# tomas-gr/RawNanoporeSignalCompression

Hardware: AMD Instinct MI355X
Metric: MSamples/s encode+decode (1/2/4/8 GPU) at fixed ratio; % HBM roofline (higher is better)
Workload: dtype int16; 1 GPU; configs[1]: 100000 reads x 100000 int16 samples per GPU (1 chunk each), C5 encode+decode; reads_per_gpu=100000, samples_per_read=100000, global_reads=100000, parallelism=dp1 (reads round-robin, no data-path collective)

## Files before the change

rawnanoporesignalcompression_amd/csrc/pgn_kernels.hip:

```cpp
#include <hip/hip_runtime.h>
#include <stdio.h>
#include <stdlib.h>
#include <string.h>

#include <algorithm>
#include <condition_variable>
#include <mutex>
#include <vector>

#include "../../include/pgnano_hip.h"
#include "../../include/pgnano_pod5.h"
#include "pgn_c5.h"
#include "pgn_internal.h"
#include "pgn_segment.h"
#include "pgn_stitch.h"
#include "pgn_ctc.h"
#include "pgn_crf.h"
#include "pgn_crf_post.h"
#include "pgn_qual.h"
#include "pgn_select.h"
#include "pgn_vbz.h"
#include "pgn_variants.h"
#include "pgn_zdec.h"
#include "pgn_zenc.h"
// ... 477 lines not shown
    bool ex = tot <= kAllocLimit;
    for (int s = 0; ex && s < nf; s++) {
        const int64_t b = z1::frame_content_bound(src + fo[s], (size_t)fl[s]);
        ex = b >= 0 && (uint64_t)b >= cs[s];
    }
    *sum = tot;
    *maxClaim = mx;
    *expand = ex;
    return true;
}
__host__ __device__ inline bool claims_pass_chunk(const uint8_t* src, uint64_t len, int nf, uint32_t n, uint64_t* sum)
{
    uint64_t mx = 0;
    bool ex = false;
    if (!blob_claims(src, len, nf, sum, &mx, &ex) || !ex) return false;
    return *sum + kVbzPadding > inter_cap(n) || mx > n;
}

__global__ void claim_scan_kernel(const uint8_t* in, const uint64_t* inOffsets, const uint64_t* inSizes,
                                  const uint32_t* counts, size_t n, int nf, uint32_t* list, uint32_t* hdr)
{
    for (size_t i = (size_t)blockIdx.x * blockDim.x + threadIdx.x; i < n; i += (size_t)gridDim.x * blockDim.x) {
        uint64_t sum = 0;
        if (!claims_pass_chunk(in + inOffsets[i], inSizes[i], nf, counts[i], &sum)) continue;
        list[atomicAdd(hdr + 4, 1u)] = (uint32_t)i;
        const uint64_t kib = (sum + 1023) >> 10;
        atomicMax(hdr + 5, kib < 0xFFFFFFFFull ? (uint32_t)kib : 0xFFFFFFFFu);
    }
}

__device__ inline int c5_parse_chunk(const uint8_t* in, uint64_t src0, uint64_t len, DecUnit* u, size_t interCap)
{
    const uint8_t* src = in + src0;
    uint64_t pos = 0;
    uint64_t cs[5];
    for (int s = 0; s < kStreams; s++) {
        uint64_t fl;
        if (s < 4) {
            if (pos > len || len - pos < 8) return PGN_ERR_CORRUPT;
            fl = ld64u(src + pos);
            pos += 8;
            if (fl > len - pos) return PGN_ERR_CORRUPT;
        } else {
            fl = len - pos;
        }
        bool ok = false;
        cs[s] = z1::frame_content_size(src + pos, (size_t)fl, &ok);
        if (!ok) return PGN_ERR_NOT_ZSTD;
        u[s].src = src0 + pos;
        u[s].len = (uint32_t)fl;
        pos += fl;
    }
    uint64_t off = 0;
    for (int s = 0; s < kStreams; s++) {
        if (cs[s] > kPassSamples || cs[s] > interCap - off) return over_claim_status(in, u, cs, kStreams);
        u[s].cs = (uint32_t)cs[s];
        u[s].interOff = (uint32_t)off;
        off += cs[s];
    }
    return PGN_OK;
}

__global__ __launch_bounds__(64) void dec_parse_kernel(DecArgs a)
{
    const size_t g = (size_t)blockIdx.x * 64 + lane_id();
    const size_t c = a.base + g;
    if (g >= a.G || c >= a.nchunks) return;
    a.status[c] = a.sampleCounts[c] > kPassSamples ? PGN_ERR_UNSUPPORTED
                                                   : c5_parse_chunk(a.in, a.inOffsets[c], a.inSizes[c], a.units + g * kStreams,
                                                                    inter_cap(a.capN));
}

__global__ __launch_bounds__(64) __attribute__((amdgpu_waves_per_eu(5))) void dec_zstd_kernel(DecArgs a)
{
    const int lane = lane_id();
    const DecLayout lay = dec_layout();
    uint8_t* sbase = a.slotScratch + (size_t)blockIdx.x * a.slotBytes;
    DecScratch S;
    S.lit = sbase + lay.lit;
    S.tables = (uint32_t*)(sbase + lay.tables);
    S.htab = (uint16_t*)(sbase + lay.htab);
    S.coopCmd = nullptr;
    S.coopStg = nullptr;
    PhaseProf P;
    P.init(a.prof);
    const size_t G = a.G, units = (size_t)a.nu * G;
    uint32_t tk = 0;
    if (lane == 0) tk = atomicAdd(a.queue, 1u);
    while (true) {
        const uint32_t u = __builtin_amdgcn_readfirstlane(tk);
        if (u >= units) break;
        if (lane == 0) tk = atomicAdd(a.queue, 1u);
        const int s = a.nu == 1 ? 0 : unit_stream((uint32_t)(u / G));
        const size_t g = u % G;
        const size_t c = a.base + g;
        S.job = a.jobs ? a.jobs + (g * kStreams + (size_t)s) * kJobBytes : nullptr;
        if (S.job && lane == 0) gst<uint32_t>(&((HufJob*)S.job)->flag, 0u);
        if (c >= a.nchunks || a.status[c] != PGN_OK) continue;
        DecUnit& d = a.units[g * kStreams + s];
        const size_t cap = a.nu == 1 ? (size_t)d.cs + kVbzPadding : (size_t)d.cs;
        uint8_t* const dst = a.inter + g * a.interStride + d.interOff;
        P.mark(3);
        long r = dec_frame_fast(a.in + d.src, d.len, dst, cap, S.job, S.htab, P, sDec.hb);
        P.mark(2);
        if (r < 0) r = zstd_decompress_wave(a.in + d.src, d.len, dst, cap, S, P);
        if (lane == 0) d.dres = (int32_t)r;
        wave_sync();
    }
    P.flush();
}

constexpr int kHufFrames = 16;
#ifndef PGN_K2_PF
#define PGN_K2_PF 1
#endif
constexpr uint32_t kPf = PGN_K2_PF;
constexpr uint32_t kRing = 16 * kPf;
constexpr uint32_t kRingBlocks = kRing / 4;
constexpr uint32_t kTabStride = kJobTabUse;
constexpr uint32_t kZeroTab = 16;
constexpr size_t kHufJunkBytes = 64 * 128;
static_assert((2 * kTabStride) % 16 == 0, "frame tables stay 16-byte aligned");

__device__ __forceinline__ uint64_t shl64(uint64_t c, uint32_t e)
{
    return c << (e & 63u);
}
__device__ __forceinline__ uint32_t cnd(bool c, uint32_t a, uint32_t b)
{
    uint32_t r;
    asm volatile("v_cndmask_b32 %0, %2, %1, %3" : "=v"(r) : "v"(a), "v"(b), "s"((uint64_t)ballot(c)));
    return r;
}
__device__ __forceinline__ uint32_t pick4(bool q1, bool q2, uint32_t a, uint32_t b, uint32_t c, uint32_t d)
{
    return cnd(q2, cnd(q1, d, c), cnd(q1, b, a));
}
__device__ __forceinline__ uint32_t sel4(const uint4& v, uint32_t i)
{
    return i == 0 ? v.x : (i == 1 ? v.y : (i == 2 ? v.z : v.w));
}

__global__ __launch_bounds__(64) void dec_huf_kernel(DecArgs a)
{
    __shared__ __attribute__((aligned(16))) uint16_t tabs[kHufFrames * kTabStride + kZeroTab];
    __shared__ uint32_t ring[kRing * 64];
    const uint32_t lane = (uint32_t)lane_id();
    const size_t G = a.G;
    const uint32_t ngrp = (uint32_t)((G + kHufFrames - 1) / kHufFrames);
    const uint32_t kq = blockIdx.x / ngrp;
    if (kq >= a.nu) return;
    const int s = unit_stream(kq);
    const size_t g0 = (size_t)(blockIdx.x % ngrp) * kHufFrames;
    const uint32_t f = lane >> 2, q = lane & 3;
    const size_t g = g0 + f;
    const bool inb = g < G && a.base + g < a.nchunks;
    const HufJob* J = (const HufJob*)(a.jobs + (inb ? (g * kStreams + (size_t)s) * kJobBytes : 0));
    const uint32_t flag = inb ? gld<uint32_t>(&J->flag) : 0u;
    const uint64_t fm = ballot(flag != 0);
    if (fm == 0) return;
    if (a.hufPrio) __builtin_amdgcn_s_setprio(3);
    PhaseProf Pp;
    Pp.init(a.prof ? a.prof + (kHufProfOff - kPhases) : nullptr);
    Pp.count(0);
    Pp.count(2, (uint64_t)__builtin_popcountll(fm));
    {
        const uint32_t lt = lane < kTabStride / 8 ? lane : kTabStride / 8 - 1;
        uint4 tv[kHufFrames];
#pragma unroll
        for (int ff = 0; ff < kHufFrames; ff++) {
            const size_t gf = (fm >> (4 * ff)) & 1u ? g0 + (size_t)ff : g0;
            tv[ff] = gld<uint4>(a.jobs + (gf * kStreams + (size_t)s) * kJobBytes + sizeof(HufJob) + 16 * lt);
        }
#pragma unroll
        for (int ff = 0; ff < kHufFrames; ff++)
            if (lane < kTabStride / 8) *(uint4*)&tabs[ff * kTabStride + 8 * lane] = tv[ff];
        if (lane < kZeroTab / 2) ((uint32_t*)&tabs[kHufFrames * kTabStride])[lane] = 0u;
    }
    uint8_t* const junk = a.jobs + G * kStreams * kJobBytes + 128 * lane;
    Pp.mark(0);
    uint64_t hp = 0, dstp = 0;
    uint4 len = make_uint4(0, 0, 0, 0), prm = make_uint4(0, 11, 0, 0);
    uint32_t C2 = 0;
    if (flag) {
        hp = gld<uint64_t>(&J->hp);
        dstp = gld<uint64_t>(&J->dst);
        len = gld<uint4>(&J->len[0]);
        prm = gld<uint4>(&J->rs);
        C2 = gld<uint32_t>(&J->C2);
    }
    const uint32_t rs = prm.x, tl = prm.y, d1 = prm.z & 0xFFu, d2 = prm.z >> 8, C1 = prm.w;
    const uint32_t so = (q > 0 ? len.x : 0u) + (q > 1 ? len.y : 0u) + (q > 2 ? len.z : 0u);
    const uint32_t sl = sel4(len, q);
    const uint32_t seg = (rs + 3) / 4;
    uint32_t nsym = flag ? (q == 3 ? rs - 3 * seg : seg) : 0u;
    const uint8_t* src = (const uint8_t*)hp + 6 + so;
    uint8_t* sdst = (uint8_t*)dstp + (size_t)seg * q;
    const uint32_t lastB = (flag && sl) ? (uint32_t)gb(src + sl - 1) : 0u;
    bool bad = flag && lastB == 0;
    const bool live = flag && !bad;
    if (!live) nsym = 0;
    const uint32_t sh1 = 32 - tl, shA = sh1 + d1, shB = sh1 + d2;
    const uint64_t e = live ? (uint64_t)src + sl - 1 : (uint64_t)junk;
    const uint64_t amin = live ? ((uint64_t)src & ~(uint64_t)15) : (uint64_t)junk;
    const uint64_t gtop = e & ~(uint64_t)15;
    const uint32_t bmax = (uint32_t)((gtop - amin) >> 4);
#if PGN_K2_DIAG == 2
    auto blk = [&](uint32_t b) { return gld<uint4>((const void*)(gtop - 16ull * (b < bmax ? b : bmax) * 0)); };
#else
    auto blk = [&](uint32_t b) { return gld<uint4>((const void*)(gtop - 16ull * (b < bmax ? b : bmax))); };
#endif
    auto stage = [&](uint32_t b, const uint4& v) {
        uint32_t* r = ring + lane + 256u * (b & (kRingBlocks - 1u));
        r[0] = v.w;
        r[64] = v.z;
        r[128] = v.y;
        r[192] = v.x;
    };
    const uint32_t hb = lastB ? z1::highbit32(lastB) : 0u;
    const uint32_t i0 = (uint32_t)(e >> 2) & 3u;
    const uint32_t v0 = live ? (uint32_t)(e & 3u) * 8u + hb : 0u;
    const uint32_t totalBits = sl ? (sl - 1) * 8u + hb : 0u;
    const uint32_t ins0 = 4 - i0;
    uint32_t insb = ins0 << 8, avail = v0;
    const uint32_t laneOff = 4u * lane;
    auto ring_at = [&](uint32_t ib) -> uint32_t {
        return *(const uint32_t*)((const uint8_t*)ring + ((ib & ((kRing - 1) << 8)) | laneOff));
    };
    uint64_t C;
    uint32_t nd;
    uint4 La[kPf], Lb[kPf];
    uint32_t lb[kPf];
    auto issue = [&](uint32_t slot) {
        lb[slot] = (insb >> 10) + 2 * kPf;
        La[slot] = blk(lb[slot]);
        Lb[slot] = blk(lb[slot] + 1);
    };
    {
        uint4 b0v[2 * kPf + 2];
#pragma unroll
        for (uint32_t k = 0; k < 2 * kPf + 2; k++) b0v[k] = blk(k);
#pragma unroll
        for (uint32_t k = 0; k < kPf; k++) {
            issue(k);
            gst<uint4>(junk, make_uint4(0, 0, 0, 0));
        }
#pragma unroll
        for (uint32_t k = 0; k < 2 * kPf + 2; k++) stage(k, b0v[k]);
        const uint4 b0 = b0v[0];
        const uint32_t dw0 = sel4(b0, i0);
        C = v0 ? ((uint64_t)dw0 << (64 - v0)) : 0ull;
        nd = ring_at(insb);
        C |= shl64((uint64_t)nd, 32u - avail);
        avail += 32;
        insb += 256;
        nd = ring_at(insb);
        if (avail <= 32) {
            C |= (uint64_t)nd;
            avail += 32;
            insb += 256;
            nd = ring_at(insb);
        }
    }
    uint64_t Cadd = 0;
    auto refill = [&]() {
        const uint32_t m01 = avail <= 32 ? 1u : 0u;
        const uint32_t x = m01 ? nd : 0u;
        Cadd = shl64((uint64_t)x, 32u - avail);
        avail += m01 << 5;
        insb += m01 << 8;
        nd = ring_at(insb);
    };
    const uint32_t tbLive = f * kTabStride, tbZero = kHufFrames * kTabStride;
    uint32_t tb = tbLive, tc1 = C1 + tbLive, tc2 = C2 + tbLive, s1 = sh1;
    auto symbol = [&](bool merge) -> uint32_t {
        const uint32_t hi = (uint32_t)(C >> 32);
        const uint32_t a0 = ((hi >> s1) + tb) << 1, a1 = ((hi >> shA) + tc1) << 1, a2 = ((hi >> shB) + tc2) << 1;
        const uint32_t am = a0 < a1 ? a0 : a1;
#if PGN_K2_DIAG == 3
        const uint32_t ent = ((am < a2 ? am : a2) & 0xFF00u) | (4u + (hi >> 30));
#else
        const uint32_t ent = *(const uint16_t*)((const uint8_t*)tabs + (am < a2 ? am : a2));
#endif
        C = shl64(merge ? (C | Cadd) : C, ent);
        avail -= ent & 0xFFu;
        return ent;
    };
    auto word4 = [&]() -> uint32_t {
        const uint32_t e0 = symbol(true);
        const uint32_t e1 = symbol(false);
        refill();
        const uint32_t e2 = symbol(true);
        const uint32_t e3 = symbol(false);
        refill();
        return __builtin_amdgcn_perm(e1, e0, 0x0C0C0501u) | __builtin_amdgcn_perm(e3, e2, 0x05010C0Cu);
    };
    auto freeze = [&](bool fz) {
        tb = fz ? tbZero : tbLive;
        tc1 = fz ? tbZero : C1 + tbLive;
        tc2 = fz ? tbZero : C2 + tbLive;
        s1 = fz ? 28u : sh1;
    };
    const uint32_t h = (16u - ((uint32_t)(uintptr_t)sdst & 15u)) & 15u;
    uint8_t* A0 = sdst + h;
    const uint32_t rb = h & 3u;
    const bool q1 = (h >> 2) & 1u, q2 = (h >> 3) & 1u;
    const uint32_t m0 = ((128u - ((uint32_t)(uintptr_t)A0 & 127u)) & 127u) >> 4;
    const int sft = 7 - (int)m0;
    const int sg = (int)(nsym / 16);
    const int nD = sg - 1;
    uint32_t P[4] = {0, 0, 0, 0}, F[4] = {0, 0, 0, 0};
    auto active = [&](int gi) { const int li = gi - sft; return li >= 0 && li < sg; };
    auto iteration = [&](int gi) -> uint4 {
        stage(lb[0], La[0]);
        stage(lb[0] + 1, Lb[0]);
#pragma unroll
        for (uint32_t k = 0; k + 1 < kPf; k++) {
            lb[k] = lb[k + 1];
            La[k] = La[k + 1];
            Lb[k] = Lb[k + 1];
        }
        issue(kPf - 1);
        uint32_t W[4];
#pragma unroll
        for (int k = 0; k < 4; k++) W[k] = word4();
        const uint32_t X0 = pick4(q1, q2, P[0], P[1], P[2], P[3]), X1 = pick4(q1, q2, P[1], P[2], P[3], W[0]),
                       X2 = pick4(q1, q2, P[2], P[3], W[0], W[1]), X3 = pick4(q1, q2, P[3], W[0], W[1], W[2]),
                       X4 = pick4(q1, q2, W[0], W[1], W[2], W[3]);
        const uint4 D = make_uint4(__builtin_amdgcn_alignbyte(X1, X0, rb), __builtin_amdgcn_alignbyte(X2, X1, rb),
                                   __builtin_amdgcn_alignbyte(X3, X2, rb), __builtin_amdgcn_alignbyte(X4, X3, rb));
        const bool act = active(gi);
        if (gi < 8) {
            const bool first = gi == sft;
#pragma unroll
            for (int k = 0; k < 4; k++) F[k] = cnd(first, W[k], F[k]);
        }
#pragma unroll
        for (int k = 0; k < 4; k++) P[k] = cnd(act, W[k], P[k]);
        freeze(!active(gi + 1));
        return D;
    };
    freeze(!active(0));
#pragma unroll
    for (int gi = 0; gi < 8; gi++) {
        const uint4 D = iteration(gi);
        const int m = gi - sft - 1;
#if PGN_K2_DIAG == 1
        uint8_t* ad = junk;
#else
        uint8_t* ad = (m >= 0 && m < nD) ? A0 + 16 * m : junk;
#endif
        gst<uint4>(ad, D);
    }
#pragma unroll
    for (int k = 1; k < 8; k++) gst<uint4>(junk + 16 * k, make_uint4(0, 0, 0, 0));
    const int lines = nD > (int)m0 ? (nD - (int)m0 + 7) / 8 : 0;
    const int trips = (int)wave_max((uint32_t)lines);
    Pp.mark(1);
    Pp.count(1, (uint64_t)trips);
    Pp.count(3, (uint64_t)wave_sum(nsym));
    for (int t = 0; t < trips; t++) {
        uint4 Dk[8];
#pragma unroll
        for (int k = 0; k < 8; k++) Dk[k] = iteration(8 + 8 * t + k);
#pragma unroll
        for (int k = 0; k < 8; k++) {
            const int m = (int)m0 + 8 * t + k;
#if PGN_K2_DIAG == 1
            uint8_t* ad = junk + 16 * k;
#else
            uint8_t* ad = m < nD ? A0 + 16 * m : junk + 16 * k;
#endif
            gst<uint4>(ad, Dk[k]);
        }
    }
    Pp.mark(2);
#pragma unroll
    for (uint32_t k = 0; k < kPf; k++) {
        stage(lb[k], La[k]);
        stage(lb[k] + 1, Lb[k]);
    }
    freeze(false);
    C |= Cadd;
    Cadd = 0;
    if (sg > 0) {
        for (uint32_t b = 0; b < h; b++) gst<uint8_t>(sdst + b, (uint8_t)(sel4(make_uint4(F[0], F[1], F[2], F[3]), b >> 2) >> (8 * (b & 3))));
        const uint32_t J16 = 16 * (uint32_t)sg - 16;
        for (uint32_t b = h; b < 16; b++)
            gst<uint8_t>(sdst + J16 + b, (uint8_t)(sel4(make_uint4(P[0], P[1], P[2], P[3]), b >> 2) >> (8 * (b & 3))));
    }
    for (uint32_t i = 16 * (uint32_t)sg; i < nsym; i++) {
        const uint32_t ent = symbol(true);
        refill();
        gst<uint8_t>(sdst + i, (uint8_t)(ent >> 8));
    }
    if (live) bad = (v0 + 32u * ((insb >> 8) - ins0) - avail) != totalBits;
    const uint64_t bm = ballot(bad);
    if (q == 0 && flag && ((bm >> (4 * f)) & 0xFull)) gst<int32_t>(&a.units[g * kStreams + (size_t)s].dres, (int32_t)z1::kDecErrHufStream);
    Pp.mark(3);
    Pp.flush();
}

__global__ __launch_bounds__(64 * kCoopWaves) void dec_huf_wide_kernel(DecArgs a)
{
    const uint32_t u = blockIdx.x;
    const size_t G = a.G;
    if ((size_t)u >= (size_t)a.nu * G) return;
    const int s = unit_stream((uint32_t)(u / G));
    const size_t g = u % G;
    if (a.base + g >= a.nchunks) return;
    const HufJob* J = (const HufJob*)(a.jobs + (g * kStreams + (size_t)s) * kJobBytes);
    if (gld<uint32_t>(&J->flag) == 0) return;
    __shared__ uint32_t stgAll[kCoopWaves * kCoopStgWords];
    __shared__ uint32_t bad;
    const uint32_t tid = threadIdx.x;
    const int wid = (int)__builtin_amdgcn_readfirstlane((int)(tid >> 6));
    const uint64_t hp = gld<uint64_t>(&J->hp), dstp = gld<uint64_t>(&J->dst);
    const uint4 len = gld<uint4>(&J->len[0]);
    const uint4 prm = gld<uint4>(&J->rs);
    const uint32_t C2 = gld<uint32_t>(&J->C2);
    const uint32_t rs = prm.x, tl = prm.y, d1 = prm.z & 0xFFu, d2 = prm.z >> 8, C1 = prm.w;
    const uint16_t* ct = (const uint16_t*)(a.jobs + (g * kStreams + (size_t)s) * kJobBytes + sizeof(HufJob));
    for (uint32_t p = tid; p < (1u << tl); p += 64 * kCoopWaves) {
        const uint32_t i1 = (p >> d1) + C1, i2 = (p >> d2) + C2;
        uint32_t i = p < i1 ? p : i1;
        i = i < i2 ? i : i2;
        const uint32_t c = gld<uint16_t>(ct + i);
        sDec.tab[p] = (uint16_t)((c >> 8) | ((c & 0xFFu) << 8));
    }
    if (tid == 0) bad = 0;
    __syncthreads();
    PhaseProf P;
    P.init(nullptr);
    const size_t remain = 6 + (size_t)len.x + len.y + len.z + len.w;
    const bool ok = huf_decode1of4_wave64(tl, (const uint8_t*)hp, remain, (uint8_t*)dstp, rs, len.x | (len.y << 16), len.z,
                                          wid, (lds_u32*)&stgAll[wid * kCoopStgWords + 2 * 64], P);
    if (!ok && lane_id() == 0) atomicOr(&bad, 1u);
    __syncthreads();
    if (tid == 0 && bad) gst<int32_t>(&a.units[g * kStreams + (size_t)s].dres, (int32_t)z1::kDecErrHufStream);
}

constexpr size_t kCoopMaxChunks = 64;
__global__ __launch_bounds__(64 * kCoopWaves) void dec_zstd_coop_kernel(DecArgs a)
{
    const int lane = lane_id();
    const int wid = (int)__builtin_amdgcn_readfirstlane(threadIdx.x >> 6);
    const size_t G = a.G;
    const uint32_t u = blockIdx.x;
    if ((size_t)u >= (size_t)a.nu * G) return;
    const int s = a.nu == 1 ? 0 : unit_stream((uint32_t)(u / G));
    const size_t g = u % G;
    const size_t c = a.base + g;
    if (c >= a.nchunks) return;
    __shared__ int32_t parseRc;
    __shared__ DecUnit myUnit;
    if (a.coopParse) {
        if (threadIdx.x == 0) {
            DecUnit uu[kStreams];
            const int rc = a.sampleCounts[c] > kPassSamples ? PGN_ERR_UNSUPPORTED
                                                            : c5_parse_chunk(a.in, a.inOffsets[c], a.inSizes[c], uu,
                                                                             inter_cap(a.capN));
            parseRc = rc;
            if (rc == PGN_OK) myUnit = uu[s];
            if (s == 0) {
                a.status[c] = rc;
                if (rc == PGN_OK) {
                    for (int k = 0; k < kStreams; k++) {
                        DecUnit& w = a.units[g * kStreams + k];
                        w.src = uu[k].src;
                        w.len = uu[k].len;
                        w.cs = uu[k].cs;
                        w.interOff = uu[k].interOff;
                    }
                }
            }
        }
        __syncthreads();
        if (parseRc != PGN_OK) return;
    } else {
        if (a.status[c] != PGN_OK) return;
        if (threadIdx.x == 0) myUnit = a.units[g * kStreams + s];
        __syncthreads();
    }
    PhaseProf P;
    P.init(a.prof);
    __shared__ uint32_t stgAll[kCoopWaves * kCoopStgWords];
    __shared__ CoopCmd cmdLds;
    lds_cmd* cmd = (lds_cmd*)&cmdLds;
    lds_u32* stg = (lds_u32*)&stgAll[wid * kCoopStgWords + 2 * 64];
    if (wid != 0) {
        coop_helper_wave(wid, cmd, stg, P);
        P.flush();
        return;
    }
    const DecLayout lay = dec_layout();
    uint8_t* sbase = a.slotScratch + (size_t)u * a.slotBytes;
    DecScratch S;
    S.lit = sbase + lay.lit;
    S.tables = (uint32_t*)(sbase + lay.tables);
    S.htab = (uint16_t*)(sbase + lay.htab);
    S.coopCmd = cmd;
    S.coopStg = stg;
    S.job = nullptr;
    const uint64_t dsrc = myUnit.src;
    const uint32_t dlen = myUnit.len, dcs = myUnit.cs, doff = myUnit.interOff;
    const size_t cap = a.nu == 1 ? (size_t)dcs + kVbzPadding : (size_t)dcs;
    const long r = zstd_decompress_wave<true>(a.in + dsrc, dlen, a.inter + g * a.interStride + doff, cap, S, P);
    if (lane == 0) a.units[g * kStreams + s].dres = (int32_t)r;
    coop_finish(cmd);
    P.flush();
}

template <class T>
__device__ __forceinline__ void dec_merge_body(const DecArgs& a, MergeLds& W)
{
    const size_t g = blockIdx.x;
    const size_t c = a.base + g;
    if (g >= a.G || c >= a.nchunks) return;
    if (a.status[c] != PGN_OK) return;
    PhaseProf P;
    P.init(a.prof);
#if PGN_MERGE_DIAG == 1
    const size_t gi = g % 32;
#else
    const size_t gi = g;
#endif
    const DecUnit* d = a.units + gi * kStreams;
    uint64_t total = 0;
    int st = PGN_OK;
    for (int s = 0; s < kStreams; s++) {
        if (d[s].dres < 0) st = PGN_ERR_ZSTD_DECOMPRESS;
        total += d[s].cs;
    }
    if (st == PGN_OK) {
        uint64_t consumed = 0;
        const int bad = c5_merge_wave(a.inter + gi * a.interStride, total, (uint64_t)d[1].dres, (uint64_t)d[2].dres,
                                      (uint64_t)d[3].dres, out_chunk<T>(a, c), a.sampleCounts[c], &consumed, W,
                                      cal_chunk<T>(a, c));
        if (bad) st = PGN_ERR_CORRUPT;
        else if (consumed != total) st = PGN_ERR_REMAINING;
    }
    if (lane_id() == 0) a.status[c] = st;
    P.mark(6);
    P.flush();
}

__global__ __launch_bounds__(64) __attribute__((amdgpu_waves_per_eu(6))) void dec_merge_kernel(DecArgs a)
{
    static __shared__ MergeLds W;
    dec_merge_body<int16_t>(a, W);
}
template <class T>
__global__ __launch_bounds__(64) __attribute__((amdgpu_waves_per_eu(6))) void dec_merge_pa_kernel(DecArgs a)
{
    static __shared__ MergeLds W;
    dec_merge_body<T>(a, W);
}

constexpr size_t kMergeWgMaxChunks = 64;

constexpr int kMergeRanges = 32;
template <class T>
__device__ __forceinline__ void dec_merge_lb_body(const DecArgs& a, MergeLds& W)
{
    const size_t g = blockIdx.x / kMergeRanges;
    const uint32_t r = blockIdx.x % kMergeRanges;
    const size_t c = a.base + g;
    if (g >= a.G || c >= a.nchunks) return;
    if (a.status[c] != PGN_OK) return;
    const uint32_t lane = (uint32_t)lane_id();
#if PGN_MERGE_DIAG == 1
    const size_t gi = g % 32;
#else
    const size_t gi = g;
#endif
    const DecUnit* d = a.units + gi * kStreams;
    uint64_t total = 0;
    int st = PGN_OK;
    for (int s = 0; s < kStreams; s++) {
        if (d[s].dres < 0) st = PGN_ERR_ZSTD_DECOMPRESS;
        total += d[s].cs;
    }
    if (st != PGN_OK) {
        if (r == 0 && lane == 0) a.status[c] = st;
        return;
    }
    uint64_t* lb = a.lookback + g * (3 * kMergeRanges);
    const uint64_t ep = a.epoch;
    const uint32_t n = a.sampleCounts[c];
    const uint8_t* in = a.inter + g * a.interStride;
    T* out = out_chunk<T>(a, c);
    const uint64_t dS = (uint64_t)d[1].dres, dM = (uint64_t)d[2].dres, dLl = (uint64_t)d[3].dres;
    const uint64_t kl = ((uint64_t)n + 3) / 4;
    const uint64_t ps = kl, pm = kl + dS, pl = kl + dS + dM, ph = kl + dS + dM + dLl;
    const uint32_t steps = (n + kSplitStep - 1) / kSplitStep;
    const uint32_t s0 = (uint32_t)((uint64_t)steps * r / kMergeRanges), s1 = (uint32_t)((uint64_t)steps * (r + 1) / kMergeRanges);
    const uint32_t t0 = s0 * kSplitStep, t1 = s1 * kSplitStep < n ? s1 * kSplitStep : n;
    uint32_t cS = 0, cM = 0, cL = 0;
    if (kl <= total) c5_class_counts(in, n, t0, t1, cS, cM, cL);
    if (lane == 0) lb_publish(lb + 3 * r, ep, (uint64_t)cS | ((uint64_t)cM << 16) | ((uint64_t)cL << 32));
    const uint64_t pc = lb_wait(lb, 0, r, ep);
    const uint64_t sN0 = wave_sum64(pc & 0xFFFFu), mN0 = wave_sum64((pc >> 16) & 0xFFFFu), lN0 = wave_sum64(pc >> 32);
    const uint64_t sN1 = sN0 + cS, mN1 = mN0 + cM, lN1 = lN0 + cL;
    const bool inside = kl <= total && ps + ((sN1 + 1) >> 1) <= total && pm + mN1 <= total && pl + lN1 <= total &&
                        ph + lN1 <= total;
    uint32_t sum = 0;
    if (inside) sum = c5_range_delta_sum(in, ps, pm, pl, ph, sN0, sN1, mN0, mN1, lN0, lN1);
    if (lane == 0) lb_publish(lb + 3 * r + 1, ep, (uint64_t)sum | ((uint64_t)(inside ? 0u : 1u) << 32));
    const uint64_t ps_ = lb_wait(lb, 1, r, ep);
    const uint32_t carryIn = (uint32_t)wave_sum64(ps_ & 0xFFFFu);
    const bool outsideBefore = wave_sum64((ps_ >> 32) & 1u) != 0;
    int bad = (!inside || outsideBefore) ? 1 : 0;
    if (!bad) {
        uint32_t carry = carryIn;
        uint64_t lEnd = 0;
        bad = c5_merge_range<false>(in, total, dS, dM, dLl, out, n, t0, t1, sN0, mN0, lN0, carry, &lEnd, W, cal_chunk<T>(a, c));
    }
    if (lane == 0) lb_publish(lb + 3 * r + 2, ep, (uint64_t)(bad ? 1u : 0u));
    if (r == kMergeRanges - 1) {
        const uint64_t dn = lb_wait(lb, 2, kMergeRanges, ep);
        const bool badAny = wave_sum64(dn & 1u) != 0;
        const uint64_t lTot = lN1;
        if (lane == 0) {
            __threadfence();
            a.status[c] = badAny ? PGN_ERR_CORRUPT : ((ph + lTot != total) ? PGN_ERR_REMAINING : PGN_OK);
        }
    }
}

__global__ __launch_bounds__(64) void dec_merge_lb_kernel(DecArgs a)
{
    __shared__ MergeLds W;
    dec_merge_lb_body<int16_t>(a, W);
}
template <class T>
__global__ __launch_bounds__(64) void dec_merge_lb_pa_kernel(DecArgs a)
{
    __shared__ MergeLds W;
    dec_merge_lb_body<T>(a, W);
}


__global__ __launch_bounds__(64) void vbz_split_kernel(EncArgs a)
{
    static __shared__ VbzSplitLds W;
    const size_t g = blockIdx.x;
    const size_t c = a.base + g;
    if (g >= a.G || c >= a.nchunks) return;
    PhaseProf P;
    P.init(a.prof);
    const uint32_t n = a.sampleCounts[c];
    uint32_t* sz = a.sizes + g * kStreams;
    if (n > kPassSamples) {
        if (lane_id() == 0) {
            sz[0] = ~0u;
            a.status[c] = PGN_ERR_UNSUPPORTED;
            a.outSizes[c] = 0;
        }
        return;
    }
    const uint32_t pad = (16u - (svb_key_length(n) & 15u)) & 15u;
    const uint32_t m = vbz_split_wave(a.samples + a.sampleOffsets[c], n, a.streams + g * kChunkStreamBytes + pad, W);
    if (lane_id() == 0) {
        sz[0] = m;
        sz[1] = pad;
    }
    P.mark(0);
    P.flush();
}

__global__ __launch_bounds__(64) void vbz_assemble_kernel(EncArgs a)
{
    const size_t g = blockIdx.x;
    const size_t c = a.base + g;
    if (g >= a.G || c >= a.nchunks) return;
    const int lane = lane_id();
    const uint32_t* sz = a.sizes + g * kStreams;
    if (sz[0] == ~0u) return;
    const uint32_t fs = a.fsizes[g * kStreams];
    const bool ok = fs <= a.outCaps[c];
    if (ok) wave_copy(a.out + a.outOffsets[c], a.frames + g * kChunkFrameBytes, fs);
    if (lane == 0) {
        a.status[c] = ok ? PGN_OK : PGN_ERR_ZSTD_COMPRESS;
        a.outSizes[c] = ok ? fs : 0;
        if (a.stats) {
            for (int s = 0; s < PGN_STATS_PER_CHUNK; s++) a.stats[c * PGN_STATS_PER_CHUNK + s] = 0;
            a.stats[c * PGN_STATS_PER_CHUNK] = sz[0];
            a.stats[c * PGN_STATS_PER_CHUNK + 5] = fs;
        }
    }
}

__global__ __launch_bounds__(64) void vbz_parse_kernel(DecArgs a)
{
// ... 2843 lines not shown
```

Measured before the change: 241,800 MSamples/s.

## Decode unaligned Huffman head bytes first, then store aligned words without byte shuffling

The Huffman decode inner loop no longer realigns each 16-byte group with pick4/alignbyte against the previous group. Instead, the unaligned head bytes are decoded up front with scalar byte stores, so later groups land directly on 16-byte-aligned addresses. The main loop is split into a fully-active phase with no per-iteration freeze or active checks and a strided line pointer, plus a tail phase that keeps masking. This cuts ALU and register pressure in the hot loop. The cost is a short divergent scalar prologue and more complex trip-count logic.

```diff
diff --git a/rawnanoporesignalcompression_amd/csrc/pgn_kernels.hip b/rawnanoporesignalcompression_amd/csrc/pgn_kernels.hip
--- a/rawnanoporesignalcompression_amd/csrc/pgn_kernels.hip
+++ b/rawnanoporesignalcompression_amd/csrc/pgn_kernels.hip
@@ -803,16 +803,13 @@
         s1 = fz ? 28u : sh1;
     };
     const uint32_t h = (16u - ((uint32_t)(uintptr_t)sdst & 15u)) & 15u;
+    const uint32_t hh = h < nsym ? h : nsym;
     uint8_t* A0 = sdst + h;
-    const uint32_t rb = h & 3u;
-    const bool q1 = (h >> 2) & 1u, q2 = (h >> 3) & 1u;
     const uint32_t m0 = ((128u - ((uint32_t)(uintptr_t)A0 & 127u)) & 127u) >> 4;
     const int sft = 7 - (int)m0;
-    const int sg = (int)(nsym / 16);
-    const int nD = sg - 1;
-    uint32_t P[4] = {0, 0, 0, 0}, F[4] = {0, 0, 0, 0};
+    const int sg = (int)((nsym - hh) / 16);
     auto active = [&](int gi) { const int li = gi - sft; return li >= 0 && li < sg; };
-    auto iteration = [&](int gi) -> uint4 {
+    auto advance = [&]() {
         stage(lb[0], La[0]);
         stage(lb[0] + 1, Lb[0]);
 #pragma unroll
@@ -822,58 +819,82 @@
             Lb[k] = Lb[k + 1];
         }
         issue(kPf - 1);
+    };
+    {
+        advance();
+        const uint32_t hmax = wave_max(hh);
+        for (uint32_t j = 0; j < hmax; j += 2) {
+            freeze(j >= hh);
+            const uint32_t e0 = symbol(true);
+            freeze(j + 1 >= hh);
+            const uint32_t e1 = symbol(false);
+            refill();
+            if (j < hh) gst<uint8_t>(sdst + j, (uint8_t)(e0 >> 8));
+            if (j + 1 < hh) gst<uint8_t>(sdst + j + 1, (uint8_t)(e1 >> 8));
+        }
+        gst<uint4>(junk, make_uint4(0, 0, 0, 0));
+    }
+    auto iteration = [&](int gi, bool all) -> uint4 {
+        advance();
         uint32_t W[4];
 #pragma unroll
         for (int k = 0; k < 4; k++) W[k] = word4();
-        const uint32_t X0 = pick4(q1, q2, P[0], P[1], P[2], P[3]), X1 = pick4(q1, q2, P[1], P[2], P[3], W[0]),
-                       X2 = pick4(q1, q2, P[2], P[3], W[0], W[1]), X3 = pick4(q1, q2, P[3], W[0], W[1], W[2]),
-                       X4 = pick4(q1, q2, W[0], W[1], W[2], W[3]);
-        const uint4 D = make_uint4(__builtin_amdgcn_alignbyte(X1, X0, rb), __builtin_amdgcn_alignbyte(X2, X1, rb),
-                                   __builtin_amdgcn_alignbyte(X3, X2, rb), __builtin_amdgcn_alignbyte(X4, X3, rb));
-        const bool act = active(gi);
-        if (gi < 8) {
-            const bool first = gi == sft;
-#pragma unroll
-            for (int k = 0; k < 4; k++) F[k] = cnd(first, W[k], F[k]);
-        }
-#pragma unroll
-        for (int k = 0; k < 4; k++) P[k] = cnd(act, W[k], P[k]);
-        freeze(!active(gi + 1));
-        return D;
+        if (!all) freeze(!active(gi + 1));
+        return make_uint4(W[0], W[1], W[2], W[3]);
     };
     freeze(!active(0));
 #pragma unroll
-    for (int gi = 0; gi < 8; gi++) {
-        const uint4 D = iteration(gi);
-        const int m = gi - sft - 1;
+    for (int gi = 0; gi < 7; gi++) {
+        const uint4 D = iteration(gi, false);
+        const int m = gi - sft;
 #if PGN_K2_DIAG == 1
         uint8_t* ad = junk;
 #else
-        uint8_t* ad = (m >= 0 && m < nD) ? A0 + 16 * m : junk;
+        uint8_t* ad = (m >= 0 && m < sg) ? A0 + 16 * m : junk;
 #endif
         gst<uint4>(ad, D);
     }
 #pragma unroll
     for (int k = 1; k < 8; k++) gst<uint4>(junk + 16 * k, make_uint4(0, 0, 0, 0));
-    const int lines = nD > (int)m0 ? (nD - (int)m0 + 7) / 8 : 0;
+    const int lines = sg > (int)m0 ? (sg - (int)m0 + 7) / 8 : 0;
     const int trips = (int)wave_max((uint32_t)lines);
+    const int tripsAll = trips - (int)wave_max((uint32_t)(sg > 0 ? trips - (sg - (int)m0) / 8 : 0));
+    uint8_t* line = sg > 0 ? A0 + 16 * m0 : junk;
+    const uint32_t lineStep = sg > 0 ? 128u : 0u;
     Pp.mark(1);
     Pp.count(1, (uint64_t)trips);
     Pp.count(3, (uint64_t)wave_sum(nsym));
-    for (int t = 0; t < trips; t++) {
+    for (int t = 0; t < tripsAll; t++) {
         uint4 Dk[8];
 #pragma unroll
-        for (int k = 0; k < 8; k++) Dk[k] = iteration(8 + 8 * t + k);
+        for (int k = 0; k < 8; k++) Dk[k] = iteration(0, true);
+#pragma unroll
+        for (int k = 0; k < 8; k++) {
+#if PGN_K2_DIAG == 1
+            uint8_t* ad = junk + 16 * k;
+#else
+            uint8_t* ad = line + 16 * k;
+#endif
+            gst<uint4>(ad, Dk[k]);
+        }
+        line += lineStep;
+    }
+    freeze(!active(7 + 8 * tripsAll));
+    for (int t = tripsAll; t < trips; t++) {
+        uint4 Dk[8];
+#pragma unroll
+        for (int k = 0; k < 8; k++) Dk[k] = iteration(7 + 8 * t + k, false);
 #pragma unroll
         for (int k = 0; k < 8; k++) {
             const int m = (int)m0 + 8 * t + k;
 #if PGN_K2_DIAG == 1
             uint8_t* ad = junk + 16 * k;
 #else
-            uint8_t* ad = m < nD ? A0 + 16 * m : junk + 16 * k;
+            uint8_t* ad = m < sg ? line + 16 * k : junk + 16 * k;
 #endif
             gst<uint4>(ad, Dk[k]);
         }
+        line += lineStep;
     }
     Pp.mark(2);
 #pragma unroll
@@ -884,13 +905,7 @@
     freeze(false);
     C |= Cadd;
     Cadd = 0;
-    if (sg > 0) {
-        for (uint32_t b = 0; b < h; b++) gst<uint8_t>(sdst + b, (uint8_t)(sel4(make_uint4(F[0], F[1], F[2], F[3]), b >> 2) >> (8 * (b & 3))));
-        const uint32_t J16 = 16 * (uint32_t)sg - 16;
-        for (uint32_t b = h; b < 16; b++)
-            gst<uint8_t>(sdst + J16 + b, (uint8_t)(sel4(make_uint4(P[0], P[1], P[2], P[3]), b >> 2) >> (8 * (b & 3))));
-    }
-    for (uint32_t i = 16 * (uint32_t)sg; i < nsym; i++) {
+    for (uint32_t i = hh + 16 * (uint32_t)sg; i < nsym; i++) {
         const uint32_t ent = symbol(true);
         refill();
         gst<uint8_t>(sdst + i, (uint8_t)(ent >> 8));
```

Result: faster. 244,400 MSamples/s, median of 6 (+1.1%).
